# mcahny/vps

Measured on AMD Instinct MI355X. Metric: frames/sec FuseTrack 1024x2048, higher is better.
Workload: dtype f32-grade: f16x3 split operands (fp16 pair with scaled residual, 22 significand bits) on MFMA, f32 accumulate

## Files before the change

### include/vps_hip.h

```cpp
#ifndef VPS_HIP_H
#define VPS_HIP_H

#include <stdint.h>

#ifdef __cplusplus
extern "C" {
#endif

int vps_abi_version(void);
const char* vps_build_info(void);

enum { VPS_ACT_NONE = 0, VPS_ACT_RELU = 1, VPS_ACT_LEAKY = 2 };
enum { VPS_PREC_F32 = 0, VPS_PREC_BF16 = 1, VPS_PREC_BF16X3 = 2, VPS_PREC_BF16X6 = 3, VPS_PREC_F16X3 = 4 };

typedef struct vps_conv_desc {
    const float* in;
    int32_t N, H, W;
    int32_t in_ld;
    int32_t in_coff;
    int32_t cin_pad;
    const float* w;
    int32_t cout, cout_pad, kpad;
    int32_t KH, KW, stride;
    int32_t pad_y[2], pad_x[2];
// ... 42 lines not shown
                    int act, float slope, void* stream);
int vps_correlation_f16(const float* in1, int ld1, int coff1, const float* in2, int ld2, int coff2,
                        float* out, int out_ld, int out_coff, int N, int H, int W, int C,
                        int max_disp, int stride2, int act, float slope, int32_t* status, void* stream);

int vps_flow_warp(const float* in, int in_ld, int in_coff, const float* flow, int flow_ld, int flow_coff,
                  float* out, int out_ld, int out_coff, int N, int H, int W, int C, void* stream);

int vps_nchw_to_nhwc(const float* in, float* out, int out_ld, int out_coff, int N, int C, int H, int W,
                     int Cpad, void* stream);
int vps_nhwc_to_nchw(const float* in, int in_ld, int in_coff, float* out, int N, int C, int H, int W, void* stream);

int vps_resize(const float* in, int in_ld, int in_coff, int Hi, int Wi,
               float* out, int out_ld, int out_coff, int Ho, int Wo,
               int N, int C, int mode, float alpha, void* stream);
int vps_pool3x3s2(const float* in, int in_ld, int in_coff, int Hi, int Wi,
                  float* out, int out_ld, int out_coff, int N, int C, int mode, void* stream);
int vps_bfp_gather(const float* const* levels, const int* ld, const int* ratio, int nlevels,
                   float* out, int out_ld, int out_coff, int N, int H0, int W0, int C, void* stream);
int vps_bfp_scatter(const float* bsf, int bsf_ld, const float* level, int lvl_ld, float* out, int out_ld,
                    int N, int H0, int W0, int C, int ratio, void* stream);
int vps_bfp_scatter_all(const float* bsf, int bsf_ld, const float* const* levels, const int* lvl_ld, float* const* outs,
                        const int* out_ld, int nlevels, int N, int H0, int W0, int C, void* stream);
int vps_axpb(const float* in, int in_ld, int in_coff, float* out, int out_ld, int out_coff,
             int64_t npix, int C, float a, float b, void* stream);

int vps_flow_prep(const float* img, const float* ref, const float* mean3, const float* std3,
                  float* out, int out_ld, int H, int W, double* partial, int nblk, float* rgb_mean_out,
                  void* stream);
int vps_flow_prep_pad(const float* img, const float* ref, const float* mean3, const float* std3,
// ... 143 lines not shown
```

### vps_amd/csrc/conv_mfma.hip

```cpp
#include "conv_common.h"

namespace {
template <int TM, int TN, int WAVES_M, int WAVES_N, bool DEFORM>
__global__ __launch_bounds__(256, 2)
void conv_mfma_f32_kernel(const vps_conv_desc d, const int M, const int tiles_m, const int tiles_n,
                          const int ksteps_per_split) {
    constexpr int BN = WAVES_N * TN * 32;
    static_assert(WAVES_M * TM * 32 == BM, "block M tile must be 128");
    static_assert(WAVES_M * WAVES_N == 4, "4 wavefronts per block");
    constexpr int NB = BN / 32;

    __shared__ __attribute__((aligned(16))) float As[BM * LDS_LD];
    __shared__ __attribute__((aligned(16))) float Bs[BN * LDS_LD];

    const int t = threadIdx.x;
    int swz = xcd_swizzle(blockIdx.x, gridDim.x);
    int tile_n, tile_m, cls, split;
    decode_tile(d, swz, tiles_n, tiles_m, tile_n, tile_m, cls, split);

    const int py = cls / d.os_x, px = cls - py * d.os_x;
    const int pad_y = d.pad_y[py], pad_x = d.pad_x[px];
    const float* __restrict__ wcls = d.w + (size_t)cls * d.cout_pad * d.kpad;

    const int H = d.H, W = d.W, KH = d.KH, KW = d.KW, cin_pad = d.cin_pad;
// ... 622 lines not shown
                                const int pos = ((w + 1) * NMF) / (NW + 1);
                                if (mf == (pos < 1 ? 1 : pos)) {
                                    __builtin_amdgcn_sched_barrier(0);
                                    work(w);
                                    __builtin_amdgcn_sched_barrier(0);
                                }
                            }
                        }
        }
        __syncthreads();
    }
    report_range<MODE>(d, amax);
    conv_epilogue<TM, TN, BN, true>(d, acc, tiles_m * BM, tile_m, tile_n, cls, split, py, px, wm, wn, lane, (cls * tiles_m + tile_m) * tiles_n + tile_n);
}

template <int V>
__global__ __launch_bounds__(256)
void conv_splitk_reduce_kernel(const vps_conv_desc d, const int M) {
    const int cv = d.cout / V;
    const size_t total = (size_t)d.nclass * M * cv;
    const size_t plane = (size_t)d.nclass * M * d.cout_pad;
    for (size_t idx = (size_t)blockIdx.x * blockDim.x + threadIdx.x; idx < total;
         idx += (size_t)gridDim.x * blockDim.x) {
        const int co = (int)(idx % cv) * V;
        const size_t t2 = idx / cv;
        const int m = (int)(t2 % M);
        const int cls = (int)(t2 / M);
        const float* __restrict__ wp = d.ws + ((size_t)cls * M + m) * d.cout_pad + co;
        float s[V];
#pragma unroll
        for (int e = 0; e < V; ++e) s[e] = 0.f;
        for (int sp0 = 0; sp0 < d.ksplit; sp0 += 8) {
            float v[8][V];
// ... 30 lines not shown
                r[0] = t[0]; r[1] = t[1]; r[2] = t[2]; r[3] = t[3];
            } else {
                r[0] = d.res[rpix * d.res_ld + d.res_coff + co];
            }
        }
        float o[V];
#pragma unroll
        for (int e = 0; e < V; ++e) {
            float v = s[e] * (d.scale ? d.scale[co + e] : 1.f) + (d.shift ? d.shift[co + e] : 0.f);
            if (d.res) v += r[e];
            o[e] = vps_act(v, d.act, d.slope);
        }
        float* op = d.out + opix * d.out_ld + d.out_coff + co;
        if constexpr (V == 4) *reinterpret_cast<f32x4*>(op) = f32x4{o[0], o[1], o[2], o[3]};
        else op[0] = o[0];
    }
}

template <int TM, int TN, int WAVES_M, int WAVES_N>
void launch_conv(const vps_conv_desc& d, const conv_plan& p, hipStream_t s) {
    const dim3 grid(p.grid), block(p.block);
    if (p.kernel == CONV_K_HALO) {
        with_prec<true>(d.prec, [&](auto mode) {
            constexpr int MODE = decltype(mode)::value;
            if (d.KH == 3) hipLaunchKernelGGL((conv_mfma_bf16h_kernel<TM, TN, WAVES_M, WAVES_N, MODE, 3, 3>), grid, block, 0, s, d, p.tiles_m, p.tiles_n, p.chunks_per_split);
            else hipLaunchKernelGGL((conv_mfma_bf16h_kernel<TM, TN, WAVES_M, WAVES_N, MODE, 2, 2>), grid, block, 0, s, d, p.tiles_m, p.tiles_n, p.chunks_per_split);
        });
        return;
    }
#define VPS_CONV_LAUNCH(KERNEL) hipLaunchKernelGGL((KERNEL), grid, block, 0, s, d, p.M, p.tiles_m, p.tiles_n, p.per_split)
// ... 58 lines not shown
            break;
        case CONV_K_N16T: case CONV_K_N32: case CONV_K_N16: vpsi_launch_conv_n16(d, p, s); break;
        case CONV_K_H8S2: vpsi_launch_conv_h8s2(d, p, s); break;
        case CONV_K_H8P: vpsi_launch_conv_h8p(d, p, s); break;
        case CONV_K_H8: vpsi_launch_conv_h8(d, p, s); break;
        case CONV_K_PW: vpsi_launch_conv_pw(d, p, s); break;
        case CONV_K_Q: vpsi_launch_conv_q(d, p, s); break;
        default:
            if (d.tile_n == 128) launch_conv<2, 2, 2, 2>(d, p, s);
            else if (d.tile_n == 64) launch_conv<2, 1, 2, 2>(d, p, s);
            else launch_conv<1, 1, 4, 1>(d, p, s);
    }
    int st = vps_launch_status();
    if (st || !p.needs_reduce) return st;
    const size_t total = (size_t)d.nclass * p.M * d.cout;
    if (p.reduce_v4) hipLaunchKernelGGL(conv_splitk_reduce_kernel<4>, dim3(stream_grid((long)(total / 4), 256)), dim3(256), 0, s, d, p.M);
    else hipLaunchKernelGGL(conv_splitk_reduce_kernel<1>, dim3(stream_grid((long)total, 256)), dim3(256), 0, s, d, p.M);
    return vps_launch_status();
}
```

### vps_amd/csrc/conv_plan.cpp

```cpp
#include "conv_plan.h"
#include <stdint.h>

namespace {

constexpr int BM = 128, BK = 32;

inline int cdiv(long a, long b) { return (int)((a + b - 1) / b); }
inline size_t in_bytes(const vps_conv_desc& d) { return (size_t)d.N * d.H * d.W * d.in_ld * sizeof(float); }
inline size_t out_bytes(const vps_conv_desc& d) { return (size_t)d.N * d.Ho * d.Wo * d.out_ld * sizeof(float); }
inline bool two_plane(int prec) { return prec == VPS_PREC_F16X3 || prec == VPS_PREC_BF16X3 || prec == VPS_PREC_BF16; }

constexpr int H8_MIN_CHUNKS = 3;
constexpr int PW_MIN_ROUNDS = 2;

conv_plan fail(conv_plan p, int n) { p.kernel = CONV_K_NONE; p.err = VPS_EARG(n); return p; }

conv_plan plan_small(const vps_conv_desc& d, conv_plan p) {
    p.block = 256;
    p.G = 1; p.logG = 0;
    while (p.G < 64 && p.G < (d.cin_pad >> 2)) { p.G <<= 1; ++p.logG; }
    const size_t wbytes = (size_t)(d.cout <= 2 ? 2 : 4) * d.kpad * sizeof(float);
    if (d.KH == 3 && d.KW == 3 && d.stride == 1 && d.nclass == 1 && d.pad_y[0] == 1 && d.pad_x[0] == 1 && d.Ho == d.H && d.Wo == d.W &&
        wbytes <= 150 * 1024 && (d.cout <= 2 || d.cout_pad >= 4) && in_bytes(d) < 0xFFFFFFF0ull &&
        (long)d.N * d.H * d.W < 0x7fffffffL) {
// ... 82 lines not shown
int vpsi_conv_check(const vps_conv_desc& d) {
    if (!d.in || !d.out) return VPS_EARG(2);
    if (d.prec < VPS_PREC_F32 || d.prec > VPS_PREC_F16X3) return VPS_EARG(12);
    if (d.prec == VPS_PREC_F32 ? !d.w : !d.w_split) return VPS_EARG(13);
    if ((d.in_ld & 3) || (d.in_coff & 3) || (d.cin_pad & 3) || d.cin_pad <= 0) return VPS_EARG(3);
    if ((d.kpad % BK) || d.kpad < d.KH * d.KW * d.cin_pad || (d.korder != 0 && d.korder != 1)) return VPS_EARG(4);
    if (d.korder == 1 && d.kpad != d.KH * d.KW * ((d.cin_pad + BK - 1) / BK) * BK) return VPS_EARG(14);
    if (d.tile_n != 32 && d.tile_n != 64 && d.tile_n != 128 && !(d.tile_n == 256 && d.offset && d.prec == VPS_PREC_F16X3 && d.korder == 1)) return VPS_EARG(5);
    if (d.cout_pad % d.tile_n || d.cout > d.cout_pad || d.cout <= 0) return VPS_EARG(6);
    if (d.nclass != d.os_y * d.os_x || d.nclass < 1 || d.os_y > 2 || d.os_x > 2) return VPS_EARG(7);
    if (d.ksplit < 1 || (d.ksplit > 1 && !d.ws)) return VPS_EARG(8);
    if (d.offset && (d.nclass != 1 || d.off_ld < 2 * d.KH * d.KW || d.KH * d.KW > 9 || d.H > 65535 || d.W > 65535)) return VPS_EARG(9);
    if (d.offset && d.prec != VPS_PREC_F32 && d.korder != 1) return VPS_EARG(17);
    if (((uintptr_t)d.in & 15) || ((uintptr_t)d.w & 15) || ((uintptr_t)d.w_split & 15)) return VPS_EARG(10);
    if (d.prec != VPS_PREC_F32 && in_bytes(d) >= 0xFFFFFFF0ull) return VPS_EARG(16);
    if (d.gn_stats && (!d.offset || d.prec == VPS_PREC_F32 || d.ksplit != 1 || d.gn_rep < 1 || (d.gn_rep & (d.gn_rep - 1)) || (d.gn_cpg != 4 && (d.gn_cpg < 8 || (d.gn_cpg & 7))) || d.cout % d.gn_cpg ||
                       ((d.cout | d.out_ld | d.out_coff) & 3) || ((uintptr_t)d.out & 15) || d.res || ((uintptr_t)d.gn_stats & 7)))
        return VPS_EARG(15);
    const long Ml = (long)d.N * d.Qh * d.Qw;
    if (Ml <= 0 || Ml > 0x7fffffffL) return VPS_EARG(11);
    return 0;
}

conv_plan vpsi_conv_plan(const vps_conv_desc& d, const conv_limits& lim, const conv_switches& sw) {
    conv_plan p = {};
    const int M = p.M = (int)((long)d.N * d.Qh * d.Qw);
    if (d.cout <= 4 && d.prec == VPS_PREC_F32 && !d.offset && d.ksplit == 1 && d.tile_n == 32) return plan_small(d, p);
    if (plan_thin(d, lim, sw, p)) return p;

    const int BN = d.tile_n;
    const int tiles_m = p.tiles_m = cdiv(M, BM);
// ... 59 lines not shown
```

### vps_amd/csrc/nn_ops.hip

```cpp
#include "common.h"

typedef float f32x4 __attribute__((ext_vector_type(4)));

namespace {

template <int V> struct vecn { typedef float type; };
template <> struct vecn<4> { typedef f32x4 type; };

template <int V>
__global__ __launch_bounds__(256)
void resize_kernel(const float* __restrict__ in, int in_ld, int in_coff, int Hi, int Wi,
                   float* __restrict__ out, int out_ld, int out_coff, int Ho, int Wo,
                   int N, int C, int mode, float alpha, float sh, float sw) {
    typedef typename vecn<V>::type vt;
    const int cv = C / V;
    const long total = (long)N * Ho * Wo * cv;
    for (long idx = (long)blockIdx.x * blockDim.x + threadIdx.x; idx < total; idx += (long)gridDim.x * blockDim.x) {
        const int c = (int)(idx % cv) * V;
        const int pix = (int)(idx / cv);
        const int x = pix % Wo;
        const int yy = pix / Wo;
        const int y = yy % Ho, n = yy / Ho;
        const float* ib = in + (size_t)n * Hi * Wi * in_ld + in_coff + c;
        vt v;
        if (mode == 1) {
            const int ys = min((int)floorf((float)y * sh), Hi - 1);
            const int xs = min((int)floorf((float)x * sw), Wi - 1);
            v = *reinterpret_cast<const vt*>(ib + ((size_t)ys * Wi + xs) * in_ld);
        } else {
            float sy = sh * ((float)y + 0.5f) - 0.5f; if (sy < 0.f) sy = 0.f;
            float sx = sw * ((float)x + 0.5f) - 0.5f; if (sx < 0.f) sx = 0.f;
            const int y0 = min((int)sy, Hi - 1), x0 = min((int)sx, Wi - 1);
            const int yp = y0 < Hi - 1 ? 1 : 0, xp = x0 < Wi - 1 ? 1 : 0;
            const float ly = sy - (float)y0, lx = sx - (float)x0;
            const float hy = 1.f - ly, hx = 1.f - lx;
            const vt p00 = *reinterpret_cast<const vt*>(ib + ((size_t)y0 * Wi + x0) * in_ld);
            const vt p01 = *reinterpret_cast<const vt*>(ib + ((size_t)y0 * Wi + x0 + xp) * in_ld);
            const vt p10 = *reinterpret_cast<const vt*>(ib + ((size_t)(y0 + yp) * Wi + x0) * in_ld);
            const vt p11 = *reinterpret_cast<const vt*>(ib + ((size_t)(y0 + yp) * Wi + x0 + xp) * in_ld);
            v = hy * (hx * p00 + lx * p01) + ly * (hx * p10 + lx * p11);
        }
        *reinterpret_cast<vt*>(out + (size_t)pix * out_ld + out_coff + c) = v * alpha;
    }
}

template <int V>
__global__ __launch_bounds__(256)
void pool3x3s2_kernel(const float* __restrict__ in, int in_ld, int in_coff, int Hi, int Wi,
                      float* __restrict__ out, int out_ld, int out_coff, int Ho, int Wo, int N, int C, int mode) {
    typedef typename vecn<V>::type vt;
    const int cv = C / V;
    const long total = (long)N * Ho * Wo * cv;
    for (long idx = (long)blockIdx.x * blockDim.x + threadIdx.x; idx < total; idx += (long)gridDim.x * blockDim.x) {
        const int c = (int)(idx % cv) * V;
// ... 229 lines not shown
        double gs = 0.0, gq = 0.0;
        for (int k = 0; k < ppb; ++k)
            for (int j = 0; j < cpg; ++j) {
                gs += ssum[k * C + t * cpg + j];
                gq += ssq[k * C + t * cpg + j];
            }
        atomicAdd(&stats[2 * t], gs);
        atomicAdd(&stats[2 * t + 1], gq);
    }
}

__global__ __launch_bounds__(256)
void groupnorm_apply4_kernel(const float* __restrict__ in, int in_ld, float* __restrict__ out, int out_ld, int out_coff, long npix,
                             int C, int G, const float* __restrict__ gamma, const float* __restrict__ beta, float eps,
                             int relu, const double* __restrict__ stats_g, int nrep) {
    __shared__ double stats[512];
    __shared__ float sc_t[256], bi_t[256];
    for (int i = threadIdx.x; i < 2 * G; i += blockDim.x) {
        double a = 0.0;
        for (int r = 0; r < nrep; ++r) a += stats_g[(size_t)r * 2 * G + i];
        stats[i] = a;
    }
    __syncthreads();
    const int c4n = C >> 2;
    const long total = npix * c4n;
    const int cpg = C / G;
    const double cnt = (double)npix * cpg;
    for (int c = threadIdx.x; c < C; c += blockDim.x) {
        const int g = c / cpg;
        const double mean = stats[2 * g] / cnt;
        double var = stats[2 * g + 1] / cnt - mean * mean;
        if (var < 0.0) var = 0.0;
        const float rstd = (float)(1.0 / sqrt(var + (double)eps));
        const float sc = rstd * gamma[c];
        const float bi = -sc * (float)mean + beta[c];
        sc_t[c] = sc; bi_t[c] = bi;
    }
    __syncthreads();
    for (long idx = (long)blockIdx.x * blockDim.x + threadIdx.x; idx < total; idx += (long)gridDim.x * blockDim.x) {
        const int c = (int)(idx % c4n) * 4;
        const long pix = idx / c4n;
        const f32x4 x = *reinterpret_cast<const f32x4*>(in + (size_t)pix * in_ld + c);
        f32x4 y;
#pragma unroll
        for (int e = 0; e < 4; ++e) {
            const float sc = sc_t[c + e], bi = bi_t[c + e];
            float v = x[e] * sc + bi;
            if (relu) v = v > 0.f ? v : 0.f;
            y[e] = v;
        }
        *reinterpret_cast<f32x4*>(out + (size_t)pix * out_ld + out_coff + c) = y;
    }
}

__global__ __launch_bounds__(256)
void tcea_temporal_kernel(const float* __restrict__ emb, int emb_ld, const float* __restrict__ emb_ref, int ref_ld,
                          const float* __restrict__ fea0, int f0_ld, const float* __restrict__ fea1, int f1_ld,
                          float* __restrict__ out, int out_ld, long npix, int C) {
    const int lane = threadIdx.x & 63, wave = threadIdx.x >> 6;
    const int c4n = C >> 2;
    for (long pix = (long)blockIdx.x * 4 + wave; pix < npix; pix += (long)gridDim.x * 4) {
        float cor0 = 0.f, cor1 = 0.f;
        for (int c4 = lane; c4 < c4n; c4 += 64) {
            const f32x4 r = *reinterpret_cast<const f32x4*>(emb_ref + (size_t)pix * ref_ld + 4 * c4);
            const f32x4 e0 = *reinterpret_cast<const f32x4*>(emb + (size_t)pix * emb_ld + 4 * c4);
// ... 42 lines not shown
            const float s = 1.f / (1.f + expf(-a[e]));
            o[e] = f[e] * s * 2.f + d[e];
        }
        *reinterpret_cast<f32x4*>(out + (size_t)pix * out_ld + c) = o;
    }
}

}

extern "C" int vps_resize(const float* in, int in_ld, int in_coff, int Hi, int Wi, float* out, int out_ld, int out_coff,
                          int Ho, int Wo, int N, int C, int mode, float alpha, void* stream) {
    if (!in || !out || N <= 0 || C <= 0 || Hi <= 0 || Wi <= 0 || Ho <= 0 || Wo <= 0) return VPS_EARG(1);
    const float sh = (float)Hi / (float)Ho, sw = (float)Wi / (float)Wo;
    if ((long)N * Ho * Wo > 0x7fffffffL) return VPS_EARG(2);
    if (!((C | in_ld | in_coff | out_ld | out_coff) & 3))
        hipLaunchKernelGGL(resize_kernel<4>, dim3(stream_grid((long)N * Ho * Wo * (C >> 2), 256)), dim3(256), 0, (hipStream_t)stream,
                           in, in_ld, in_coff, Hi, Wi, out, out_ld, out_coff, Ho, Wo, N, C, mode, alpha, sh, sw);
    else
        hipLaunchKernelGGL(resize_kernel<1>, dim3(stream_grid((long)N * Ho * Wo * C, 256)), dim3(256), 0, (hipStream_t)stream,
                           in, in_ld, in_coff, Hi, Wi, out, out_ld, out_coff, Ho, Wo, N, C, mode, alpha, sh, sw);
    return vps_launch_status();
}

extern "C" int vps_pool3x3s2(const float* in, int in_ld, int in_coff, int Hi, int Wi, float* out, int out_ld, int out_coff,
                             int N, int C, int mode, void* stream) {
    if (!in || !out || N <= 0 || C <= 0 || Hi <= 0 || Wi <= 0) return VPS_EARG(1);
    const int Ho = (Hi + 2 - 3) / 2 + 1, Wo = (Wi + 2 - 3) / 2 + 1;
    if ((long)N * Ho * Wo > 0x7fffffffL) return VPS_EARG(2);
    if (!((C | in_ld | in_coff | out_ld | out_coff) & 3))
        hipLaunchKernelGGL(pool3x3s2_kernel<4>, dim3(stream_grid((long)N * Ho * Wo * (C >> 2), 256)), dim3(256), 0, (hipStream_t)stream,
                           in, in_ld, in_coff, Hi, Wi, out, out_ld, out_coff, Ho, Wo, N, C, mode);
    else
        hipLaunchKernelGGL(pool3x3s2_kernel<1>, dim3(stream_grid((long)N * Ho * Wo * C, 256)), dim3(256), 0, (hipStream_t)stream,
                           in, in_ld, in_coff, Hi, Wi, out, out_ld, out_coff, Ho, Wo, N, C, mode);
    return vps_launch_status();
// ... 123 lines not shown
```

### vps_amd/detector.py

```python
import os
import os.path as osp
import warnings

import numpy as np
import torch
import torch.nn as nn

from . import hip, nhwc, panoptic_ops
from . import registry as R
from .base import HipModule
from .flownet2 import FlowNet2
from .panoptic_ops import MaskRemoval, MaskROI, panoptic_combine

_BOARD = []


def announce(pairs):
    _BOARD[:] = [(a, b) for a, b in pairs][:2]



def _np(a):
    return a.cpu().numpy() if torch.is_tensor(a) else np.asarray(a)

# ... 284 lines not shown
                ref_bsf = cache['cat'].window(0, C)
            elif self.reuse_ref_features and iid >= 0 and is_first:
                ref_bsf = cat.window(0, C)
            else:
                with ws.scope():
                    rl = self.neck.run(self.backbone.run(nhwc.from_nchw(ref_img, ws, 'ref_nhwc'), ws, 'rbb.'), ws, 'rfpn.')
                ref_bsf = self.extra_neck.gather(rl, ws, 'neck.refcat').window(0, C)
                self._mark('ref_backbone_fpn')
            self._cache = dict(iid=iid, cat=cat, shape=(H, W), probe=self._probe(img), slot=None if pf is None else pf.get('slot'))
            x, aux = self.extra_neck.run(levels, cat, ref_bsf, ws, 'neck.')
            self._mark('extra_neck')
        sem_done = None
        if side is not None:
            side.wait_stream(main)
            with torch.cuda.stream(side):
                fcn_score = self.panopticFPN.run(x[0:self.panopticFPN.num_levels], ws)
                sem_done = torch.cuda.Event()
                sem_done.record(side)
        else:
            fcn_score = self.panopticFPN.run(x[0:self.panopticFPN.num_levels], ws)
        if inject is not None and 'fcn_score' in inject:
            fcn_score = nhwc.from_nchw(inject['fcn_score'].to(dev), ws, 'inj.fcn_score')
        self._mark('semantic_head')
        if self.with_fusion and late and main is not None:
            self._pf = (self._pf or []) + [self._enqueue_image_stages(late[0][0], late[0][1], main, defer_backbone=self.defer_backbone)]
        nprop = None
        if inject is not None and 'proposals' in inject:
            proposals = inject['proposals'].to(dev)
        else:
            proposals, nprop = self.rpn_head.run(x, ws, meta['img_shape'], self.test_cfg.rpn)
        self._mark('rpn')
        det = self.simple_test_bboxes(x, meta, proposals, im_info, is_first, ws, inject, defer_tracking, nprop)
        self._mark('bbox_track')

        det_bboxes, det_labels = det['det_bboxes'], det['det_labels']
# ... 289 lines not shown
```

### vps_amd/heads.py

```python
import numpy as np
import torch
import torch.nn as nn

from . import hip, nhwc
from .base import HipModule
from .necks import _ConvModule
from .registry import HEADS, PANOPTIC, ROI_EXTRACTORS


class _DeformConvParams(nn.Module):

    def __init__(self, cin, cout, k):
        super().__init__()
        self.weight = nn.Parameter(torch.empty(cout, cin, k, k).normal_(0, 0.01))
        self.stride, self.padding = (1, 1), (1, 1)
        self.bias = None


class _DeformConvWithOffset(nn.Module):
    def __init__(self, cin, cout):
        super().__init__()
        self.conv_offset = nn.Conv2d(cin, 18, 3, padding=1)
        self.conv = _DeformConvParams(cin, cout, 3)

# ... 11 lines not shown
            _DeformConvWithOffset(in_channels, out_channels), nn.GroupNorm(32, out_channels), nn.ReLU(),
            _DeformConvWithOffset(out_channels, out_channels), nn.GroupNorm(32, out_channels), nn.ReLU())])
        self.conv_pred = _ConvModule(out_channels * 4, num_classes, 1)

    def pack(self, device):
        seq = self.deform_convs[0]
        self._tower = []
        for ci, gi in ((0, 1), (3, 4), (6, 7)):
            d, g = seq[ci], seq[gi]
            self._tower.append(dict(
                off=nhwc.pack_conv_module(d.conv_offset, device=device),
                dcn=nhwc.PackedConv(d.conv.weight, None, None, 1, 1, device=device, deform=True),
                gamma=g.weight.detach().float().to(device), beta=g.bias.detach().float().to(device), eps=g.eps, G=g.num_groups))
        self._pred = nhwc.pack_conv_module(self.conv_pred.conv, device=device)

    def run(self, levels, ws, tag='sem.'):
        self.ensure_packed(levels[0].t.device)
        assert len(levels) == self.num_levels
        l0 = levels[0]
        oc = self.out_channels
        cat = ws.fmap(tag + 'cat', l0.N, l0.H, l0.W, oc * len(levels), temp=True)
        stats = ws.get(tag + 'gnstats', (len(levels) * len(self._tower), nhwc.GN_REP, 64), dtype=torch.float64)
        stats.zero_()
        for li, x in enumerate(levels):
            src = x
            for ti, t in enumerate(self._tower):
                n = '%sl%dt%d' % (tag, li, ti)
                off = t['off'](x, ws=ws, name=n + 'off')
                slot = stats[li * len(self._tower) + ti]
                raw = t['dcn'](x, ws=ws, name=n + 'dcn', offset=off, gn=(slot, t['G']), temp=True)
                if x is not src:
                    ws.release(x)
                last = ti == len(self._tower) - 1
                if last and li == 0:
                    dst = cat.window(0, oc)
                else:
                    dst = ws.fmap(n + 'gn', raw.N, raw.H, raw.W, raw.C, temp=True)
                x = nhwc.groupnorm_relu(raw, dst, t['G'], t['gamma'], t['beta'], t['eps'], slot, stats_ready=t['dcn'].gn_fused)
                ws.release(raw)
            if li > 0:
                nhwc.resize(x, cat.window(li * oc, oc), 'bilinear')
                ws.release(x)
        score = self._pred(cat, ws=ws, name=tag + 'fcn_score')
        ws.release(cat)
        return score

    def forward(self, inputs):
        ws = nhwc.Workspace(inputs[0].device)
# ... 236 lines not shown
```

### vps_amd/hip.py

```python
import ctypes
import os
from ctypes import (POINTER, Structure, byref, c_char_p, c_double, c_float, c_int, c_int32, c_int64, c_uint64,
                    c_void_p)

import torch

_HERE = os.path.dirname(os.path.abspath(__file__))
LIB_PATH = os.environ.get('VPS_HIP_LIB') or os.path.join(_HERE, 'csrc', 'libvpship.so')
ABI_VERSION = 21

ACT_NONE, ACT_RELU, ACT_LEAKY = 0, 1, 2
PREC_F32, PREC_BF16, PREC_BF16X3, PREC_BF16X6, PREC_F16X3 = 0, 1, 2, 3, 4

SYMBOLS = [
    'vps_abi_version', 'vps_build_info', 'vps_conv2d', 'vps_resample2d', 'vps_channelnorm', 'vps_correlation',
    'vps_flow_warp', 'vps_nchw_to_nhwc', 'vps_nhwc_to_nchw', 'vps_resize', 'vps_pool3x3s2', 'vps_bfp_gather',
    'vps_bfp_scatter', 'vps_bfp_scatter_all', 'vps_axpb', 'vps_flow_prep', 'vps_flow_prep_pad', 'vps_flow_stage', 'vps_flow_stage_full', 'vps_groupnorm_relu', 'vps_groupnorm_apply', 'vps_tcea_temporal',
    'vps_tcea_modulate', 'vps_tcea_modulate_ld', 'vps_correlation_f16', 'vps_roi_align', 'vps_nms_batched', 'vps_delta2bbox', 'vps_bbox_overlaps',
    'vps_row_softmax', 'vps_mask_count', 'vps_mask_commit', 'vps_mask_removal', 'vps_mask_removal_dep', 'vps_mask_removal_hist', 'vps_frame_tail', 'vps_mask_level', 'vps_panoptic_combine',
    'vps_panoptic_combine_dev', 'vps_rpn_select', 'vps_rpn_collect', 'vps_maskroi_select', 'vps_maskroi_finish', 'vps_track_assign', 'vps_pan_instances',
    'vps_unify_hist', 'vps_unify_tables', 'vps_unify_write', 'vps_image_prep', 'vps_resize_u8', 'vps_segment_stats', 'vps_segment_paint', 'vps_pair_count',
    'vps_png_info', 'vps_png_decode_bgr8', 'vps_jpeg_info', 'vps_jpeg_decode_coef', 'vps_jpeg_reconstruct',
    'vps_png_encode_bound', 'vps_png_deflate',
    'vps_unify_tables_image', 'vps_segment_stats_ch', 'vps_segment_paint_ch', 'vps_sseg_confusion',
]


class ConvDesc(Structure):
    _fields_ = [
        ('inp', c_void_p), ('N', c_int32), ('H', c_int32), ('W', c_int32),
        ('in_ld', c_int32), ('in_coff', c_int32), ('cin_pad', c_int32),
# ... 69 lines not shown
    for s in SYMBOLS[2:]:
        getattr(lib, s).restype = c_int
    lib.vps_conv2d.argtypes = [POINTER(ConvDesc), c_void_p]
    lib.vps_resample2d.argtypes = [Tensor4, Tensor4, Tensor4, c_int, c_int, c_int, c_int, c_void_p]
    lib.vps_channelnorm.argtypes = [Tensor4, Tensor4, c_int, c_int, c_int, c_int, c_void_p]
    lib.vps_correlation.argtypes = [c_void_p, c_int, c_int, c_void_p, c_int, c_int, c_void_p, c_int, c_int,
                                    c_int, c_int, c_int, c_int, c_int, c_int, c_int, c_float, c_void_p]
    lib.vps_correlation_f16.argtypes = [c_void_p, c_int, c_int, c_void_p, c_int, c_int, c_void_p, c_int, c_int,
                                        c_int, c_int, c_int, c_int, c_int, c_int, c_int, c_float, c_void_p, c_void_p]
    lib.vps_flow_warp.argtypes = [c_void_p, c_int, c_int, c_void_p, c_int, c_int, c_void_p, c_int, c_int,
                                  c_int, c_int, c_int, c_int, c_void_p]
    lib.vps_nchw_to_nhwc.argtypes = [c_void_p, c_void_p, c_int, c_int, c_int, c_int, c_int, c_int, c_int, c_void_p]
    lib.vps_nhwc_to_nchw.argtypes = [c_void_p, c_int, c_int, c_void_p, c_int, c_int, c_int, c_int, c_void_p]
    lib.vps_resize.argtypes = [c_void_p, c_int, c_int, c_int, c_int, c_void_p, c_int, c_int, c_int, c_int,
                               c_int, c_int, c_int, c_float, c_void_p]
    lib.vps_pool3x3s2.argtypes = [c_void_p, c_int, c_int, c_int, c_int, c_void_p, c_int, c_int, c_int, c_int, c_int,
                                  c_void_p]
    lib.vps_bfp_gather.argtypes = [POINTER(c_void_p), POINTER(c_int), POINTER(c_int), c_int, c_void_p, c_int, c_int,
                                   c_int, c_int, c_int, c_int, c_void_p]
    lib.vps_bfp_scatter.argtypes = [c_void_p, c_int, c_void_p, c_int, c_void_p, c_int, c_int, c_int, c_int, c_int,
                                    c_int, c_void_p]
    lib.vps_bfp_scatter_all.argtypes = [c_void_p, c_int, POINTER(c_void_p), POINTER(c_int), POINTER(c_void_p), POINTER(c_int), c_int, c_int, c_int,
                                        c_int, c_int, c_void_p]
    lib.vps_axpb.argtypes = [c_void_p, c_int, c_int, c_void_p, c_int, c_int, c_int64, c_int, c_float, c_float,
                             c_void_p]
    lib.vps_flow_prep.argtypes = [c_void_p, c_void_p, c_void_p, c_void_p, c_void_p, c_int, c_int, c_int, c_void_p,
                                  c_int, c_void_p, c_void_p]
    lib.vps_flow_prep_pad.argtypes = [c_void_p, c_void_p, c_void_p, c_void_p, c_void_p, c_int, c_int, c_int, c_int, c_int, c_void_p,
                                      c_int, c_void_p, c_void_p]
    lib.vps_flow_stage.argtypes = [c_void_p, c_int, c_void_p, c_int, c_int, c_int, c_int, c_int, c_float, c_int,
# ... 108 lines not shown
```

### vps_amd/nhwc.py

```python
import ctypes
import math
import os
import weakref
from ctypes import c_float, c_int, c_void_p

import torch

from . import hip


def _ceil(a, b):
    return (a + b - 1) // b * b


_PREC_NAMES = {'f32': hip.PREC_F32, 'bf16': hip.PREC_BF16, 'bf16x3': hip.PREC_BF16X3, 'bf16x6': hip.PREC_BF16X6, 'f16x3': hip.PREC_F16X3}
PREC_NAMES = _PREC_NAMES
_PLANES = {hip.PREC_BF16: 1, hip.PREC_BF16X3: 2, hip.PREC_BF16X6: 3, hip.PREC_F16X3: 3}
MFMA_PRODUCTS = {hip.PREC_F32: 1, hip.PREC_BF16: 1, hip.PREC_BF16X3: 3, hip.PREC_BF16X6: 6, hip.PREC_F16X3: 3}
F16_SLOTS = 4096
_F16_STATUS = {}
_F16_LAYERS = {}
_F16_NEXT = [1]
F16_FALLBACKS = [0]

# ... 38 lines not shown
SMALL_ON_MFMA = os.environ.get('VPS_SMALL_MFMA', '0') != '0'
THIN_KERNEL = os.environ.get('VPS_THIN', '1') != '0'
GN_REP = 32


def check_f16_range(device):
    device = torch.device(device)
    for key, t in _F16_STATUS.items():
        if key[0] == device.type and (device.index is None or key[1] == device.index):
            if int(t.amax().item()) != 0:
                t.zero_()
                raise hip.VpsHipError('f16x3: an activation exceeded the fp16 range (|x| > 65504) in a convolution; the fp16 split is '
                                      'not fp32-grade there. Run it with prec=bf16x6 (or f32).')


class FMap:
    __slots__ = ('t', 'C', 'coff')

    def __init__(self, t, C=None, coff=0):
        assert t.dim() == 4 and t.dtype == torch.float32 and t.is_contiguous()
        self.t = t
        self.C = t.shape[3] if C is None else C
        self.coff = coff
        assert self.coff + self.C <= t.shape[3]

    N = property(lambda s: s.t.shape[0])
    H = property(lambda s: s.t.shape[1])
    W = property(lambda s: s.t.shape[2])
    ld = property(lambda s: s.t.shape[3])
    npix = property(lambda s: s.t.shape[0] * s.t.shape[1] * s.t.shape[2])

    def window(self, coff, C):
        return FMap(self.t, C, self.coff + coff)

    def ptr(self):
        return hip.ptr(self.t)

    def to_nchw(self):
        out = torch.empty(self.N, self.C, self.H, self.W, dtype=torch.float32, device=self.t.device)
        hip.check(hip.load().vps_nhwc_to_nchw(self.ptr(), self.ld, self.coff, hip.ptr(out), self.N, self.C, self.H, self.W,
                                              hip.stream_ptr()), 'vps_nhwc_to_nchw')
        return out


POOLING = os.environ.get('VPS_WS_POOL', '1') != '0'


# ... 289 lines not shown
        w[0, :M] = mat
        self.prec = DEFAULT_PREC if prec is None else prec
        self._fb, self.f16_slot = None, 0
        wscale = self._set_weights(w, mat.device)
        self.scale, self.shift, self.has_scale = None, None, False
        if wscale is not None:
            self.scale, self.has_scale = wscale[:M].contiguous(), True
        return self

    def out_hw(self, H, W):
        if self.transposed:
            return 2 * H, 2 * W
        p = self.pad_y[0]
        return (H + 2 * p - self.KH) // self.stride + 1, (W + 2 * p - self.KW) // self.stride + 1

    def __call__(self, x, out=None, ws=None, name=None, res=None, res_shift=0, offset=None, act=None, gn=None, temp=False, keep=False):
        if getattr(self, '_mfma_twin', None) is not None and x.N * x.H * x.W >= 100000:
            return self._mfma_twin(x, out, ws, name, res, res_shift, offset, act, gn, temp, keep)
        assert x.C == self.cin or (x.C >= self.cin and x.C <= self.cin_pad), (x.C, self.cin)
        assert x.coff % 4 == 0 and x.ld % 4 == 0 and x.coff + self.cin_pad <= x.ld, (x.coff, x.ld, self.cin_pad)
        Ho, Wo = self.out_hw(x.H, x.W)
        if out is None:
            out = ws.fmap(name, x.N, Ho, Wo, self.cout, temp=temp, out=keep)
        assert (out.N, out.H, out.W) == (x.N, Ho, Wo) and out.C == self.cout, ((out.N, out.H, out.W, out.C), (x.N, Ho, Wo, self.cout))
        ckey = (x.t.data_ptr(), x.N, x.H, x.W, x.ld, x.coff, out.t.data_ptr(), out.ld, out.coff,
                None if res is None else (res.t.data_ptr(), res.ld, res.coff, res_shift),
                None if offset is None else (offset.t.data_ptr(), offset.ld), act, getattr(hip.stream_ptr(), 'value', None) or 0,
                None if gn is None else (gn[0].data_ptr(), gn[1]))
        cache = self.__dict__.setdefault('_dcache', {})
        hit = cache.get(ckey)
        if hit is not None and CONV_TRACE is None:
            self.gn_fused = bool(hit[0].gn_stats)
            hip.conv2d(hit[0])
            return out
        d = hip.ConvDesc()
        d.inp = x.t.data_ptr(); d.N, d.H, d.W = x.N, x.H, x.W
        d.in_ld, d.in_coff, d.cin_pad = x.ld, x.coff, self.cin_pad
        d.prec = self.prec
        d.korder = self.korder
        if self.prec == hip.PREC_F32:
            d.w = self.w.data_ptr()
        else:
            d.w_split = self.w_split.data_ptr()
# ... 27 lines not shown
            d.status = f16_status(x.t.device).data_ptr() + 4 * getattr(self, 'f16_slot', 0)
        tiles = ((M + 127) // 128) * (self.cout_pad // tile_n) * d.nclass
        ksteps = self.kpad // 32
        ksplit = 1
        if tiles < 256 and ksteps >= 8 and not getattr(self, 'small', False):
            ksplit = max(1, min((SPLITK_TARGET_BLOCKS + tiles - 1) // tiles, ksteps // 4, 32))
            ntap = self.KH * self.KW
            if self.korder == 1:
                nch = ksteps // ntap
                ksplit = max(k for k in range(1, ksplit + 1) if -(-nch // -(-nch // k)) == k)
            else:
                per = (ksteps + ksplit - 1) // ksplit
                ksplit = (ksteps + per - 1) // per
        d.ksplit = ksplit
        self.gn_fused = False
        if gn is not None and self.deform and self.prec != hip.PREC_F32 and ksplit == 1 and res is None and not ((self.cout | out.ld | out.coff) & 3):
            cpg = self.cout // gn[1]
            if self.cout % gn[1] == 0 and (cpg == 4 or cpg % 8 == 0):
                assert gn[0].dtype == torch.float64 and gn[0].numel() == GN_REP * 2 * gn[1] and gn[0].is_contiguous()
                d.gn_stats, d.gn_cpg, d.gn_rep = gn[0].data_ptr(), cpg, GN_REP
                self.gn_fused = True
        if ksplit > 1:
            need = ksplit * d.nclass * M * self.cout_pad
            ntick = d.nclass * (self.cout_pad // tile_n) * max((M + 127) // 128, x.N * ((d.Qh + 7) // 8) * ((d.Qw + 15) // 16))
            if ws is not None:
                key = '__splitk_ws_%x' % (getattr(hip.stream_ptr(), 'value', None) or 0)
                wsb = ws.bufs.get(key)
                if wsb is None or wsb.numel() < need:
                    wsb = torch.empty(max(need, 1 << 24), dtype=torch.float32, device=x.t.device)
                    ws.bufs[key] = wsb
                tck = ws.bufs.get(key + '_tickets')
# ... 45 lines not shown
        return PackedConv(m.weight, m.bias, bnd, stride=m.stride[0], padding=m.padding[0], act=act, slope=slope,
                          transposed=True, device=device, prec=prec)
    return PackedConv(m.weight, m.bias, bnd, stride=m.stride[0], padding=m.padding[0], act=act, slope=slope,
                      device=device, deform=deform, prec=prec)


def pack_linear(weight, bias, act=hip.ACT_NONE, device='cuda', chw=None, prec=None):
    w = weight.detach().float().cpu()
    if chw is not None:
        C, S = chw
        w = w.view(w.shape[0], C, S).permute(0, 2, 1).reshape(w.shape[0], C * S)
    return PackedConv(w.view(w.shape[0], w.shape[1], 1, 1), bias, None, 1, 0, act=act, device=device, prec=prec)


def resize(x, out, mode='bilinear', alpha=1.0):
    hip.check(hip.load().vps_resize(x.ptr(), x.ld, x.coff, x.H, x.W, out.ptr(), out.ld, out.coff, out.H, out.W,
                                    x.N, x.C, 0 if mode == 'bilinear' else 1, float(alpha), hip.stream_ptr()), 'vps_resize')
    return out


def pool3x3s2(x, out, mode='max'):
    hip.check(hip.load().vps_pool3x3s2(x.ptr(), x.ld, x.coff, x.H, x.W, out.ptr(), out.ld, out.coff, x.N, x.C,
                                       0 if mode == 'max' else 1, hip.stream_ptr()), 'vps_pool3x3s2')
    return out


CORR_F16 = [os.environ.get('VPS_CORR_F16', '1') != '0']
F16_CORR_SLOT = F16_SLOTS - 1


# ... 100 lines not shown
```

Baseline: 56.20.

## Fuse GroupNorm stats into split-K reduce and apply pending norm in resize

For the semantic head tower, the last deformable conv on levels above zero now leaves its output un-normalised and marks it with a pending GroupNorm. The GN statistics are gathered in the split-K reduce kernel through per-block double sums and atomics. The scale, shift and ReLU are then applied inside the bilinear resize that upsamples the level. This drops a separate GroupNorm apply pass over the full-resolution tensor and allows GN fusion when ksplit is above one. In exchange the reduce kernel gets extra shared-memory reductions and atomics, and GN is applied to the four source pixels of each bilinear output rather than once per pixel.

```diff
diff --git a/include/vps_hip.h b/include/vps_hip.h
--- a/include/vps_hip.h
+++ b/include/vps_hip.h
@@ -80,6 +80,11 @@
 int vps_resize(const float* in, int in_ld, int in_coff, int Hi, int Wi,
                float* out, int out_ld, int out_coff, int Ho, int Wo,
                int N, int C, int mode, float alpha, void* stream);
+int vps_resize_gn(const float* in, int in_ld, int in_coff, int Hi, int Wi,
+                  float* out, int out_ld, int out_coff, int Ho, int Wo,
+                  int N, int C, int mode, float alpha,
+                  int G, const float* gamma, const float* beta, float eps, int relu,
+                  const double* stats, int nrep, void* stream);
 int vps_pool3x3s2(const float* in, int in_ld, int in_coff, int Hi, int Wi,
                   float* out, int out_ld, int out_coff, int N, int C, int mode, void* stream);
 int vps_bfp_gather(const float* const* levels, const int* ld, const int* ratio, int nlevels,
diff --git a/vps_amd/csrc/conv_mfma.hip b/vps_amd/csrc/conv_mfma.hip
--- a/vps_amd/csrc/conv_mfma.hip
+++ b/vps_amd/csrc/conv_mfma.hip
@@ -660,9 +660,12 @@
     conv_epilogue<TM, TN, BN, true>(d, acc, tiles_m * BM, tile_m, tile_n, cls, split, py, px, wm, wn, lane, (cls * tiles_m + tile_m) * tiles_n + tile_n);
 }
 
-template <int V>
+template <int V, bool GN = false>
 __global__ __launch_bounds__(256)
 void conv_splitk_reduce_kernel(const vps_conv_desc d, const int M) {
+    static_assert(!GN || V == 4, "GroupNorm sums: float4 stores");
+    __shared__ double gsum[GN ? 256 : 1], gsq[GN ? 256 : 1];
+    double ds = 0.0, dq = 0.0;
     const int cv = d.cout / V;
     const size_t total = (size_t)d.nclass * M * cv;
     const size_t plane = (size_t)d.nclass * M * d.cout_pad;
@@ -723,6 +726,25 @@
         float* op = d.out + opix * d.out_ld + d.out_coff + co;
         if constexpr (V == 4) *reinterpret_cast<f32x4*>(op) = f32x4{o[0], o[1], o[2], o[3]};
         else op[0] = o[0];
+        if constexpr (GN) {
+#pragma unroll
+            for (int e = 0; e < V; ++e) { ds += (double)o[e]; dq += (double)o[e] * (double)o[e]; }
+        }
+    }
+    if constexpr (GN) {
+        const int t = threadIdx.x;
+        gsum[t] = ds; gsq[t] = dq;
+        __syncthreads();
+        const int G = d.cout / d.gn_cpg;
+        if (t < G) {
+            const int j0 = t * d.gn_cpg / 4, j1 = j0 + d.gn_cpg / 4;
+            double s = 0.0, q = 0.0;
+            for (int k = 0; k < 256 / cv; ++k)
+                for (int j = j0; j < j1; ++j) { s += gsum[k * cv + j]; q += gsq[k * cv + j]; }
+            double* __restrict__ st = d.gn_stats + (size_t)(blockIdx.x & (d.gn_rep - 1)) * 2 * G;
+            atomicAdd(&st[2 * t], s);
+            atomicAdd(&st[2 * t + 1], q);
+        }
     }
 }
 
@@ -811,7 +833,8 @@
     int st = vps_launch_status();
     if (st || !p.needs_reduce) return st;
     const size_t total = (size_t)d.nclass * p.M * d.cout;
-    if (p.reduce_v4) hipLaunchKernelGGL(conv_splitk_reduce_kernel<4>, dim3(stream_grid((long)(total / 4), 256)), dim3(256), 0, s, d, p.M);
-    else hipLaunchKernelGGL(conv_splitk_reduce_kernel<1>, dim3(stream_grid((long)total, 256)), dim3(256), 0, s, d, p.M);
+    if (d.gn_stats) hipLaunchKernelGGL((conv_splitk_reduce_kernel<4, true>), dim3(stream_grid((long)(total / 4), 256)), dim3(256), 0, s, d, p.M);
+    else if (p.reduce_v4) hipLaunchKernelGGL((conv_splitk_reduce_kernel<4, false>), dim3(stream_grid((long)(total / 4), 256)), dim3(256), 0, s, d, p.M);
+    else hipLaunchKernelGGL((conv_splitk_reduce_kernel<1, false>), dim3(stream_grid((long)total, 256)), dim3(256), 0, s, d, p.M);
     return vps_launch_status();
 }
diff --git a/vps_amd/csrc/conv_plan.cpp b/vps_amd/csrc/conv_plan.cpp
--- a/vps_amd/csrc/conv_plan.cpp
+++ b/vps_amd/csrc/conv_plan.cpp
@@ -120,7 +120,7 @@
     if (d.offset && d.prec != VPS_PREC_F32 && d.korder != 1) return VPS_EARG(17);
     if (((uintptr_t)d.in & 15) || ((uintptr_t)d.w & 15) || ((uintptr_t)d.w_split & 15)) return VPS_EARG(10);
     if (d.prec != VPS_PREC_F32 && in_bytes(d) >= 0xFFFFFFF0ull) return VPS_EARG(16);
-    if (d.gn_stats && (!d.offset || d.prec == VPS_PREC_F32 || d.ksplit != 1 || d.gn_rep < 1 || (d.gn_rep & (d.gn_rep - 1)) || (d.gn_cpg != 4 && (d.gn_cpg < 8 || (d.gn_cpg & 7))) || d.cout % d.gn_cpg ||
+    if (d.gn_stats && (!d.offset || d.prec == VPS_PREC_F32 || (d.ksplit != 1 && (d.tile_counter || 1024 % d.cout)) || d.gn_rep < 1 || (d.gn_rep & (d.gn_rep - 1)) || (d.gn_cpg != 4 && (d.gn_cpg < 8 || (d.gn_cpg & 7))) || d.cout % d.gn_cpg ||
                        ((d.cout | d.out_ld | d.out_coff) & 3) || ((uintptr_t)d.out & 15) || d.res || ((uintptr_t)d.gn_stats & 7)))
         return VPS_EARG(15);
     const long Ml = (long)d.N * d.Qh * d.Qw;
diff --git a/vps_amd/csrc/gn_table.h b/vps_amd/csrc/gn_table.h
--- /dev/null
+++ b/vps_amd/csrc/gn_table.h
@@ -0,0 +1,32 @@
+#ifndef VPS_GN_TABLE_H
+#define VPS_GN_TABLE_H
+
+__device__ __forceinline__ void gn_scale_shift_table(const double* __restrict__ stats_g, const int nrep, const int C, const int G,
+                                                     const long npix, const float* __restrict__ gamma, const float* __restrict__ beta,
+                                                     const float eps, float* __restrict__ sc_t, float* __restrict__ bi_t) {
+    const int cpg = C / G;
+    const double cnt = (double)npix * cpg;
+    for (int c = threadIdx.x; c < C; c += blockDim.x) {
+        const int g = c / cpg;
+        double s = 0.0, q = 0.0;
+        for (int r = 0; r < nrep; ++r) {
+            s += stats_g[(size_t)r * 2 * G + 2 * g];
+            q += stats_g[(size_t)r * 2 * G + 2 * g + 1];
+        }
+        const double mean = s / cnt;
+        double var = q / cnt - mean * mean;
+        if (var < 0.0) var = 0.0;
+        const float rstd = (float)(1.0 / sqrt(var + (double)eps));
+        const float sc = rstd * gamma[c];
+        const float bi = -sc * (float)mean + beta[c];
+        sc_t[c] = sc; bi_t[c] = bi;
+    }
+}
+
+__device__ __forceinline__ float gn_affine_relu(const float x, const float sc, const float bi, const int relu) {
+    float v = x * sc + bi;
+    if (relu) v = v > 0.f ? v : 0.f;
+    return v;
+}
+
+#endif
diff --git a/vps_amd/csrc/nn_ops.hip b/vps_amd/csrc/nn_ops.hip
--- a/vps_amd/csrc/nn_ops.hip
+++ b/vps_amd/csrc/nn_ops.hip
@@ -1,4 +1,5 @@
 #include "common.h"
+#include "gn_table.h"
 
 typedef float f32x4 __attribute__((ext_vector_type(4)));
 
@@ -7,12 +8,34 @@
 template <int V> struct vecn { typedef float type; };
 template <> struct vecn<4> { typedef f32x4 type; };
 
-template <int V>
+struct ResizeGn {
+    const double* stats;
+    const float* gamma;
+    const float* beta;
+    float eps;
+    int nrep, G, relu;
+    long npix;
+};
+
+template <int V, bool GN = false>
 __global__ __launch_bounds__(256)
 void resize_kernel(const float* __restrict__ in, int in_ld, int in_coff, int Hi, int Wi,
                    float* __restrict__ out, int out_ld, int out_coff, int Ho, int Wo,
-                   int N, int C, int mode, float alpha, float sh, float sw) {
+                   int N, int C, int mode, float alpha, float sh, float sw, const ResizeGn gn = ResizeGn{}) {
     typedef typename vecn<V>::type vt;
+    static_assert(!GN || V == 4, "pending GroupNorm: float4 channel groups");
+    __shared__ float sc_t[GN ? 256 : 1], bi_t[GN ? 256 : 1];
+    if constexpr (GN) {
+        gn_scale_shift_table(gn.stats, gn.nrep, C, gn.G, gn.npix, gn.gamma, gn.beta, gn.eps, sc_t, bi_t);
+        __syncthreads();
+    }
+    auto norm = [&](vt x, const int c) -> vt {
+        if constexpr (GN) {
+#pragma unroll
+            for (int e = 0; e < 4; ++e) x[e] = gn_affine_relu(x[e], sc_t[c + e], bi_t[c + e], gn.relu);
+        }
+        return x;
+    };
     const int cv = C / V;
     const long total = (long)N * Ho * Wo * cv;
     for (long idx = (long)blockIdx.x * blockDim.x + threadIdx.x; idx < total; idx += (long)gridDim.x * blockDim.x) {
@@ -26,7 +49,7 @@
         if (mode == 1) {
             const int ys = min((int)floorf((float)y * sh), Hi - 1);
             const int xs = min((int)floorf((float)x * sw), Wi - 1);
-            v = *reinterpret_cast<const vt*>(ib + ((size_t)ys * Wi + xs) * in_ld);
+            v = norm(*reinterpret_cast<const vt*>(ib + ((size_t)ys * Wi + xs) * in_ld), c);
         } else {
             float sy = sh * ((float)y + 0.5f) - 0.5f; if (sy < 0.f) sy = 0.f;
             float sx = sw * ((float)x + 0.5f) - 0.5f; if (sx < 0.f) sx = 0.f;
@@ -34,10 +57,10 @@
             const int yp = y0 < Hi - 1 ? 1 : 0, xp = x0 < Wi - 1 ? 1 : 0;
             const float ly = sy - (float)y0, lx = sx - (float)x0;
             const float hy = 1.f - ly, hx = 1.f - lx;
-            const vt p00 = *reinterpret_cast<const vt*>(ib + ((size_t)y0 * Wi + x0) * in_ld);
-            const vt p01 = *reinterpret_cast<const vt*>(ib + ((size_t)y0 * Wi + x0 + xp) * in_ld);
-            const vt p10 = *reinterpret_cast<const vt*>(ib + ((size_t)(y0 + yp) * Wi + x0) * in_ld);
-            const vt p11 = *reinterpret_cast<const vt*>(ib + ((size_t)(y0 + yp) * Wi + x0 + xp) * in_ld);
+            const vt p00 = norm(*reinterpret_cast<const vt*>(ib + ((size_t)y0 * Wi + x0) * in_ld), c);
+            const vt p01 = norm(*reinterpret_cast<const vt*>(ib + ((size_t)y0 * Wi + x0 + xp) * in_ld), c);
+            const vt p10 = norm(*reinterpret_cast<const vt*>(ib + ((size_t)(y0 + yp) * Wi + x0) * in_ld), c);
+            const vt p11 = norm(*reinterpret_cast<const vt*>(ib + ((size_t)(y0 + yp) * Wi + x0 + xp) * in_ld), c);
             v = hy * (hx * p00 + lx * p01) + ly * (hx * p10 + lx * p11);
         }
         *reinterpret_cast<vt*>(out + (size_t)pix * out_ld + out_coff + c) = v * alpha;
@@ -297,41 +320,18 @@
 void groupnorm_apply4_kernel(const float* __restrict__ in, int in_ld, float* __restrict__ out, int out_ld, int out_coff, long npix,
                              int C, int G, const float* __restrict__ gamma, const float* __restrict__ beta, float eps,
                              int relu, const double* __restrict__ stats_g, int nrep) {
-    __shared__ double stats[512];
     __shared__ float sc_t[256], bi_t[256];
-    for (int i = threadIdx.x; i < 2 * G; i += blockDim.x) {
-        double a = 0.0;
-        for (int r = 0; r < nrep; ++r) a += stats_g[(size_t)r * 2 * G + i];
-        stats[i] = a;
-    }
+    gn_scale_shift_table(stats_g, nrep, C, G, npix, gamma, beta, eps, sc_t, bi_t);
     __syncthreads();
     const int c4n = C >> 2;
     const long total = npix * c4n;
-    const int cpg = C / G;
-    const double cnt = (double)npix * cpg;
-    for (int c = threadIdx.x; c < C; c += blockDim.x) {
-        const int g = c / cpg;
-        const double mean = stats[2 * g] / cnt;
-        double var = stats[2 * g + 1] / cnt - mean * mean;
-        if (var < 0.0) var = 0.0;
-        const float rstd = (float)(1.0 / sqrt(var + (double)eps));
-        const float sc = rstd * gamma[c];
-        const float bi = -sc * (float)mean + beta[c];
-        sc_t[c] = sc; bi_t[c] = bi;
-    }
-    __syncthreads();
     for (long idx = (long)blockIdx.x * blockDim.x + threadIdx.x; idx < total; idx += (long)gridDim.x * blockDim.x) {
         const int c = (int)(idx % c4n) * 4;
         const long pix = idx / c4n;
         const f32x4 x = *reinterpret_cast<const f32x4*>(in + (size_t)pix * in_ld + c);
         f32x4 y;
 #pragma unroll
-        for (int e = 0; e < 4; ++e) {
-            const float sc = sc_t[c + e], bi = bi_t[c + e];
-            float v = x[e] * sc + bi;
-            if (relu) v = v > 0.f ? v : 0.f;
-            y[e] = v;
-        }
+        for (int e = 0; e < 4; ++e) y[e] = gn_affine_relu(x[e], sc_t[c + e], bi_t[c + e], relu);
         *reinterpret_cast<f32x4*>(out + (size_t)pix * out_ld + out_coff + c) = y;
     }
 }
@@ -404,11 +404,24 @@
     const float sh = (float)Hi / (float)Ho, sw = (float)Wi / (float)Wo;
     if ((long)N * Ho * Wo > 0x7fffffffL) return VPS_EARG(2);
     if (!((C | in_ld | in_coff | out_ld | out_coff) & 3))
-        hipLaunchKernelGGL(resize_kernel<4>, dim3(stream_grid((long)N * Ho * Wo * (C >> 2), 256)), dim3(256), 0, (hipStream_t)stream,
-                           in, in_ld, in_coff, Hi, Wi, out, out_ld, out_coff, Ho, Wo, N, C, mode, alpha, sh, sw);
+        hipLaunchKernelGGL((resize_kernel<4, false>), dim3(stream_grid((long)N * Ho * Wo * (C >> 2), 256)), dim3(256), 0, (hipStream_t)stream,
+                           in, in_ld, in_coff, Hi, Wi, out, out_ld, out_coff, Ho, Wo, N, C, mode, alpha, sh, sw, ResizeGn{});
     else
-        hipLaunchKernelGGL(resize_kernel<1>, dim3(stream_grid((long)N * Ho * Wo * C, 256)), dim3(256), 0, (hipStream_t)stream,
-                           in, in_ld, in_coff, Hi, Wi, out, out_ld, out_coff, Ho, Wo, N, C, mode, alpha, sh, sw);
+        hipLaunchKernelGGL((resize_kernel<1, false>), dim3(stream_grid((long)N * Ho * Wo * C, 256)), dim3(256), 0, (hipStream_t)stream,
+                           in, in_ld, in_coff, Hi, Wi, out, out_ld, out_coff, Ho, Wo, N, C, mode, alpha, sh, sw, ResizeGn{});
+    return vps_launch_status();
+}
+
+extern "C" int vps_resize_gn(const float* in, int in_ld, int in_coff, int Hi, int Wi, float* out, int out_ld, int out_coff,
+                             int Ho, int Wo, int N, int C, int mode, float alpha, int G, const float* gamma, const float* beta,
+                             float eps, int relu, const double* stats, int nrep, void* stream) {
+    if (!in || !out || !gamma || !beta || !stats || N != 1 || C <= 0 || Hi <= 0 || Wi <= 0 || Ho <= 0 || Wo <= 0) return VPS_EARG(1);
+    if ((long)N * Ho * Wo > 0x7fffffffL) return VPS_EARG(2);
+    if (C > 256 || G <= 0 || C % G || nrep < 1 || ((C | in_ld | in_coff | out_ld | out_coff) & 3)) return VPS_EARG(3);
+    const float sh = (float)Hi / (float)Ho, sw = (float)Wi / (float)Wo;
+    const ResizeGn gn = {stats, gamma, beta, eps, nrep, G, relu, (long)N * Hi * Wi};
+    hipLaunchKernelGGL((resize_kernel<4, true>), dim3(stream_grid((long)N * Ho * Wo * (C >> 2), 256)), dim3(256), 0, (hipStream_t)stream,
+                       in, in_ld, in_coff, Hi, Wi, out, out_ld, out_coff, Ho, Wo, N, C, mode, alpha, sh, sw, gn);
     return vps_launch_status();
 }
 
diff --git a/vps_amd/detector.py b/vps_amd/detector.py
--- a/vps_amd/detector.py
+++ b/vps_amd/detector.py
@@ -322,11 +322,11 @@
         if side is not None:
             side.wait_stream(main)
             with torch.cuda.stream(side):
-                fcn_score = self.panopticFPN.run(x[0:self.panopticFPN.num_levels], ws)
+                fcn_score = self.panopticFPN.run(x[0:self.panopticFPN.num_levels], ws, fuse_gn=True)
                 sem_done = torch.cuda.Event()
                 sem_done.record(side)
         else:
-            fcn_score = self.panopticFPN.run(x[0:self.panopticFPN.num_levels], ws)
+            fcn_score = self.panopticFPN.run(x[0:self.panopticFPN.num_levels], ws, fuse_gn=True)
         if inject is not None and 'fcn_score' in inject:
             fcn_score = nhwc.from_nchw(inject['fcn_score'].to(dev), ws, 'inj.fcn_score')
         self._mark('semantic_head')
diff --git a/vps_amd/heads.py b/vps_amd/heads.py
--- a/vps_amd/heads.py
+++ b/vps_amd/heads.py
@@ -49,7 +49,7 @@
                 gamma=g.weight.detach().float().to(device), beta=g.bias.detach().float().to(device), eps=g.eps, G=g.num_groups))
         self._pred = nhwc.pack_conv_module(self.conv_pred.conv, device=device)
 
-    def run(self, levels, ws, tag='sem.'):
+    def run(self, levels, ws, tag='sem.', fuse_gn=False):
         self.ensure_packed(levels[0].t.device)
         assert len(levels) == self.num_levels
         l0 = levels[0]
@@ -63,10 +63,14 @@
                 n = '%sl%dt%d' % (tag, li, ti)
                 off = t['off'](x, ws=ws, name=n + 'off')
                 slot = stats[li * len(self._tower) + ti]
-                raw = t['dcn'](x, ws=ws, name=n + 'dcn', offset=off, gn=(slot, t['G']), temp=True)
+                raw = t['dcn'](x, ws=ws, name=n + 'dcn', offset=off, gn=(slot, t['G']), temp=True, gn_split=fuse_gn)
                 if x is not src:
                     ws.release(x)
                 last = ti == len(self._tower) - 1
+                if fuse_gn and last and li > 0 and t['dcn'].gn_fused:
+                    raw.pending = nhwc.PendingNorm(slot, t['G'], t['gamma'], t['beta'], t['eps'])
+                    x = raw
+                    break
                 if last and li == 0:
                     dst = cat.window(0, oc)
                 else:
diff --git a/vps_amd/hip.py b/vps_amd/hip.py
--- a/vps_amd/hip.py
+++ b/vps_amd/hip.py
@@ -14,7 +14,7 @@
 
 SYMBOLS = [
     'vps_abi_version', 'vps_build_info', 'vps_conv2d', 'vps_resample2d', 'vps_channelnorm', 'vps_correlation',
-    'vps_flow_warp', 'vps_nchw_to_nhwc', 'vps_nhwc_to_nchw', 'vps_resize', 'vps_pool3x3s2', 'vps_bfp_gather',
+    'vps_flow_warp', 'vps_nchw_to_nhwc', 'vps_nhwc_to_nchw', 'vps_resize', 'vps_resize_gn', 'vps_pool3x3s2', 'vps_bfp_gather',
     'vps_bfp_scatter', 'vps_bfp_scatter_all', 'vps_axpb', 'vps_flow_prep', 'vps_flow_prep_pad', 'vps_flow_stage', 'vps_flow_stage_full', 'vps_groupnorm_relu', 'vps_groupnorm_apply', 'vps_tcea_temporal',
     'vps_tcea_modulate', 'vps_tcea_modulate_ld', 'vps_correlation_f16', 'vps_roi_align', 'vps_nms_batched', 'vps_delta2bbox', 'vps_bbox_overlaps',
     'vps_row_softmax', 'vps_mask_count', 'vps_mask_commit', 'vps_mask_removal', 'vps_mask_removal_dep', 'vps_mask_removal_hist', 'vps_frame_tail', 'vps_mask_level', 'vps_panoptic_combine',
@@ -114,6 +114,8 @@
     lib.vps_nhwc_to_nchw.argtypes = [c_void_p, c_int, c_int, c_void_p, c_int, c_int, c_int, c_int, c_void_p]
     lib.vps_resize.argtypes = [c_void_p, c_int, c_int, c_int, c_int, c_void_p, c_int, c_int, c_int, c_int,
                                c_int, c_int, c_int, c_float, c_void_p]
+    lib.vps_resize_gn.argtypes = [c_void_p, c_int, c_int, c_int, c_int, c_void_p, c_int, c_int, c_int, c_int,
+                                  c_int, c_int, c_int, c_float, c_int, c_void_p, c_void_p, c_float, c_int, c_void_p, c_int, c_void_p]
     lib.vps_pool3x3s2.argtypes = [c_void_p, c_int, c_int, c_int, c_int, c_void_p, c_int, c_int, c_int, c_int, c_int,
                                   c_void_p]
     lib.vps_bfp_gather.argtypes = [POINTER(c_void_p), POINTER(c_int), POINTER(c_int), c_int, c_void_p, c_int, c_int,
diff --git a/vps_amd/nhwc.py b/vps_amd/nhwc.py
--- a/vps_amd/nhwc.py
+++ b/vps_amd/nhwc.py
@@ -76,14 +76,22 @@
                                       'not fp32-grade there. Run it with prec=bf16x6 (or f32).')
 
 
+class PendingNorm:
+    __slots__ = ('stats', 'G', 'gamma', 'beta', 'eps')
+
+    def __init__(self, stats, G, gamma, beta, eps):
+        self.stats, self.G, self.gamma, self.beta, self.eps = stats, G, gamma, beta, float(eps)
+
+
 class FMap:
-    __slots__ = ('t', 'C', 'coff')
-
-    def __init__(self, t, C=None, coff=0):
+    __slots__ = ('t', 'C', 'coff', 'pending')
+
+    def __init__(self, t, C=None, coff=0, pending=None):
         assert t.dim() == 4 and t.dtype == torch.float32 and t.is_contiguous()
         self.t = t
         self.C = t.shape[3] if C is None else C
         self.coff = coff
+        self.pending = pending
         assert self.coff + self.C <= t.shape[3]
 
     N = property(lambda s: s.t.shape[0])
@@ -93,6 +101,7 @@
     npix = property(lambda s: s.t.shape[0] * s.t.shape[1] * s.t.shape[2])
 
     def window(self, coff, C):
+        assert self.pending is None, 'a pending GroupNorm belongs to the whole map'
         return FMap(self.t, C, self.coff + coff)
 
     def ptr(self):
@@ -412,9 +421,12 @@
         p = self.pad_y[0]
         return (H + 2 * p - self.KH) // self.stride + 1, (W + 2 * p - self.KW) // self.stride + 1
 
-    def __call__(self, x, out=None, ws=None, name=None, res=None, res_shift=0, offset=None, act=None, gn=None, temp=False, keep=False):
+    def __call__(self, x, out=None, ws=None, name=None, res=None, res_shift=0, offset=None, act=None, gn=None, temp=False, keep=False,
+                 gn_split=False):
         if getattr(self, '_mfma_twin', None) is not None and x.N * x.H * x.W >= 100000:
-            return self._mfma_twin(x, out, ws, name, res, res_shift, offset, act, gn, temp, keep)
+            return self._mfma_twin(x, out, ws, name, res, res_shift, offset, act, gn, temp, keep, gn_split)
+        if x.pending is not None:
+            raise hip.VpsHipError('PackedConv: the input carries a pending GroupNorm and the conv loaders do not apply one; normalise it with groupnorm_relu')
         assert x.C == self.cin or (x.C >= self.cin and x.C <= self.cin_pad), (x.C, self.cin)
         assert x.coff % 4 == 0 and x.ld % 4 == 0 and x.coff + self.cin_pad <= x.ld, (x.coff, x.ld, self.cin_pad)
         Ho, Wo = self.out_hw(x.H, x.W)
@@ -424,7 +436,7 @@
         ckey = (x.t.data_ptr(), x.N, x.H, x.W, x.ld, x.coff, out.t.data_ptr(), out.ld, out.coff,
                 None if res is None else (res.t.data_ptr(), res.ld, res.coff, res_shift),
                 None if offset is None else (offset.t.data_ptr(), offset.ld), act, getattr(hip.stream_ptr(), 'value', None) or 0,
-                None if gn is None else (gn[0].data_ptr(), gn[1]))
+                None if gn is None else (gn[0].data_ptr(), gn[1], bool(gn_split)))
         cache = self.__dict__.setdefault('_dcache', {})
         hit = cache.get(ckey)
         if hit is not None and CONV_TRACE is None:
@@ -482,7 +494,8 @@
                 ksplit = (ksteps + per - 1) // per
         d.ksplit = ksplit
         self.gn_fused = False
-        if gn is not None and self.deform and self.prec != hip.PREC_F32 and ksplit == 1 and res is None and not ((self.cout | out.ld | out.coff) & 3):
+        gn_ok = ksplit == 1 or (gn_split and not SPLITK_LAST_BLOCK and 1024 % self.cout == 0)
+        if gn is not None and self.deform and self.prec != hip.PREC_F32 and gn_ok and res is None and not ((self.cout | out.ld | out.coff) & 3):
             cpg = self.cout // gn[1]
             if self.cout % gn[1] == 0 and (cpg == 4 or cpg % 8 == 0):
                 assert gn[0].dtype == torch.float64 and gn[0].numel() == GN_REP * 2 * gn[1] and gn[0].is_contiguous()
@@ -558,6 +571,12 @@
 
 
 def resize(x, out, mode='bilinear', alpha=1.0):
+    pn = x.pending
+    if pn is not None:
+        hip.check(hip.load().vps_resize_gn(x.ptr(), x.ld, x.coff, x.H, x.W, out.ptr(), out.ld, out.coff, out.H, out.W,
+                                           x.N, x.C, 0 if mode == 'bilinear' else 1, float(alpha), pn.G, hip.ptr(pn.gamma), hip.ptr(pn.beta),
+                                           pn.eps, 1, hip.ptr(pn.stats), GN_REP, hip.stream_ptr()), 'vps_resize_gn')
+        return out
     hip.check(hip.load().vps_resize(x.ptr(), x.ld, x.coff, x.H, x.W, out.ptr(), out.ld, out.coff, out.H, out.W,
                                     x.N, x.C, 0 if mode == 'bilinear' else 1, float(alpha), hip.stream_ptr()), 'vps_resize')
     return out
```

After: 56.30 (median of 6 runs). No clear change (+0.2%).
